# JTtNinjaCode/CPU-Ray-Tracing-Implementation

Hardware: AMD Instinct MI355X
Metric: Msamples/sec (pixels*spp) Cornell Box 800x800@1024spp; 1/2/4/8-GPU scaling (higher is better)
Workload: dtype fp64; 1 GPU; cornell_box 800x800 1024spp depth 50, light sampling on; key=cornell_box 800x800 1024spp depth 50 f64 pool=0 chunk=0 K=0 world=1, spp=1024, max_depth=50, tiles=16x16 round-robin over ranks, parallelism=tiles1, kernel_timing=on, rounds_per_frame=1, grid_lanes=458752

## Files before the change

### cpu-ray-tracing-implementation_amd/csrc/rt_device.h

```cpp
#pragma once

#include <hip/hip_runtime.h>
#include <stdint.h>

#include <type_traits>

#include "rt_room.h"
#include "rt_scene.h"
#include "rt_sin.h"
#include "rt_types.h"

namespace rtd {

#ifndef RT_BIG_SPHERE_R
#define RT_BIG_SPHERE_R 16
#endif
#define RT_EXT_FN __device__ __attribute__((noinline))

#ifndef RT_PRECISE_F32
__device__ __forceinline__ float fdiv(float a, float b) { return a * __builtin_amdgcn_rcpf(b); }
__device__ __forceinline__ float fsqrt(float x) { return __builtin_amdgcn_sqrtf(x); }
__device__ __forceinline__ float flog(float x) { return __builtin_amdgcn_logf(x) * 0.693147180559945309f; }
__device__ __forceinline__ float frsq(float x) { return __builtin_amdgcn_rsqf(x); }
__device__ __forceinline__ void sincos2pi(float u, float& s, float& c) {
// ... 7 lines not shown
__device__ __forceinline__ float frsq(float x) { return 1.0f / sqrtf(x); }
__device__ __forceinline__ void sincos2pi(float u, float& s, float& c) {
  float phi = 2 * 3.14159265358979f * u;
  s = sinf(phi);
  c = cosf(phi);
}
#endif
__device__ __forceinline__ double frcp(double b) {
  const double r0 = __builtin_amdgcn_rcp(b);
  double r = r0;
  double e = fma(-b, r, 1.0);
  r = fma(r, e, r);
  e = fma(-b, r, 1.0);
  r = fma(r, e, r);
  return __builtin_isfinite(r) ? r : r0;
}
__device__ __forceinline__ double fdiv(double a, double b) {
  const double r = frcp(b);
  const double q = a * r;
  const double res = fma(fma(-b, q, a), r, q);
  return __builtin_isfinite(res) ? res : q;
}
__device__ __forceinline__ double fdiv_fin(double a, double b) {
  const double r = frcp(b);
  const double q = a * r;
  return fma(fma(-b, q, a), r, q);
}
__device__ __forceinline__ double frsq(double x) {
  const double r0 = __builtin_amdgcn_rsq(x);
  const double h = 0.5 * x;
  double r = r0;
  r = r * fma(-h * r, r, 1.5);
  r = r * fma(-h * r, r, 1.5);
  return __builtin_isfinite(r) ? r : r0;
}
__device__ __forceinline__ double frsq_nz(double x) {
  const double r0 = __builtin_amdgcn_rsq(x);
  const double h = 0.5 * x;
  double r = r0;
  r = r * fma(-h * r, r, 1.5);
  r = r * fma(-h * r, r, 1.5);
  return r;
}
__device__ __forceinline__ double fsqrt01(double x) {
  const double r = __builtin_amdgcn_rsq(x);
  double g = x * r, h = 0.5 * r;
  const double e = fma(-g, h, 0.5);
  g = fma(g, e, g);
  h = fma(h, e, h);
  g = fma(fma(-g, g, x), h, g);
  return x > 0.0 ? g : 0.0;
}
__device__ __forceinline__ float fsqrt01(float x) { return fsqrt(x); }
__device__ __forceinline__ double fsqrt(double x) {
  const double r = __builtin_amdgcn_rsq(x);
  double g = x * r, h = 0.5 * r;
  const double e = fma(-g, h, 0.5);
  g = fma(g, e, g);
  h = fma(h, e, h);
  g = fma(fma(-g, g, x), h, g);
  return (x > 0.0 && x < __builtin_huge_val()) ? g : (x >= 0.0 ? x : __builtin_nan(""));
}
__device__ __forceinline__ float fdiv_inv(float a, float b, float inv_b) {
#ifndef RT_PRECISE_F32
  return a * inv_b;
#else
  return a / b;
#endif
}
__device__ __forceinline__ double fdiv_inv(double a, double b, double) { return fdiv(a, b); }
__device__ __forceinline__ double flog(double x) { return log(x); }
__device__ double2 g_sincos_tab[kSinCosTab];
__device__ __forceinline__ void sincos2pi(double u, double& s, double& c) {
  const double t = u * double(kSinCosTab);
  const double h = floor(t);
  const double2 sc = g_sincos_tab[(uint32_t)(int32_t)h & (kSinCosTab - 1)];
  const double d = (t - h) * (2.0 * 3.14159265358979323846 / kSinCosTab);
  const double d2 = d * d;
  const double sd = d * fma(d2, fma(d2, 1.0 / 120.0, -1.0 / 6.0), 1.0);
  const double cm1 = d2 * fma(d2, fma(d2, -1.0 / 720.0, 1.0 / 24.0), -0.5);
  s = fma(sc.y, sd, fma(sc.x, cm1, sc.x));
  c = fma(-sc.x, sd, fma(sc.y, cm1, sc.y));
}
__device__ __forceinline__ float div_pi(float x) { return fdiv(x, 3.14159265358979323846f); }
__device__ __forceinline__ double div_pi(double x) { return x * 0.318309886183790671537767526745; }
__device__ __forceinline__ float pow5(float x) { return (x * x) * (x * x) * x; }
__device__ __forceinline__ double pow5(double x) { return (x * x) * (x * x) * x; }

template <class R>
__device__ __forceinline__ V<R> mkv(R x, R y, R z) {
  return {x, y, z};
}
template <class R>
__device__ __forceinline__ V<R> ld3(const R* p) {
  return {p[0], p[1], p[2]};
}
template <class R>
__device__ __forceinline__ V<R> operator+(V<R> a, V<R> b) {
  return {a.x + b.x, a.y + b.y, a.z + b.z};
}
template <class R>
__device__ __forceinline__ V<R> operator-(V<R> a, V<R> b) {
  return {a.x - b.x, a.y - b.y, a.z - b.z};
}
template <class R>
__device__ __forceinline__ V<R> operator-(V<R> a) {
// ... 1215 lines not shown
  tmax = h ? th : tmax;
  best = h ? idx : best;
}
template <int A, class R>
__device__ __forceinline__ void flat_quads(const FlatQuadT<R>* q, uint32_t n, int32_t base, V<R> o, V<R> d,
                                           V<R> inv, R tmin, R& tmax, int32_t& best, uint64_t xkey) {
#pragma unroll 1
  for (uint32_t k = 0; k + 1 < n; k += 2) {
    const FlatQuad2<R> r = ld_scalar(reinterpret_cast<const FlatQuad2<R>*>(q + k));
    flat_quad_test<A>(r.a, base + (int32_t)k, o, d, inv, tmin, tmax, best, xkey);
    flat_quad_test<A>(r.b, base + (int32_t)k + 1, o, d, inv, tmin, tmax, best, xkey);
  }
  if (n & 1u) flat_quad_test<A>(ld_scalar(q + (n - 1)), base + (int32_t)(n - 1), o, d, inv, tmin, tmax, best, xkey);
}
template <class R>
struct Slab {
  R t0[3], t1[3], tn, tf, th;
};
template <class R>
__device__ __forceinline__ Slab<R> flat_slab(const FlatBoxT<R>& b, V<R> o, V<R> inv, R tmin, int32_t excl_i,
                                             uint32_t xf) {
  Slab<R> s;
  const bool left = sizeof(R) == 4 && excl_i == b.inst;
  const R ninf = -Num<R>::inf();
  auto dist = [&](R p, R oa, R ia) { return (p - oa) * ia; };
  s.t0[0] = (left & (xf == 0)) ? ninf : dist(b.lo[0], o.x, inv.x);
  s.t1[0] = (left & (xf == 1)) ? ninf : dist(b.hi[0], o.x, inv.x);
  s.t0[1] = (left & (xf == 2)) ? ninf : dist(b.lo[1], o.y, inv.y);
  s.t1[1] = (left & (xf == 3)) ? ninf : dist(b.hi[1], o.y, inv.y);
  s.t0[2] = (left & (xf == 4)) ? ninf : dist(b.lo[2], o.z, inv.z);
  s.t1[2] = (left & (xf == 5)) ? ninf : dist(b.hi[2], o.z, inv.z);
  s.tn = fmax(fmax(fmin(s.t0[0], s.t1[0]), fmin(s.t0[1], s.t1[1])), fmin(s.t0[2], s.t1[2]));
  s.tf = fmin(fmin(fmax(s.t0[0], s.t1[0]), fmax(s.t0[1], s.t1[1])), fmax(s.t0[2], s.t1[2]));
  s.th = s.tn >= tmin ? s.tn : s.tf;
  return s;
}
template <class R>
__device__ __forceinline__ RoomHit<R> flat_room_test(const FlatRoomHeadT<R>& b, V<R> o, V<R> inv, R tmin,
                                                     uint32_t excl_e, int32_t excl_i) {
  auto dist = [&](R p, R oa, R ia) { return (p - oa) * ia; };
  R t0[3] = {dist(b.lo[0], o.x, inv.x), dist(b.lo[1], o.y, inv.y), dist(b.lo[2], o.z, inv.z)};
  R t1[3] = {dist(b.hi[0], o.x, inv.x), dist(b.hi[1], o.y, inv.y), dist(b.hi[2], o.z, inv.z)};
  if constexpr (sizeof(R) == 4) {
    const bool left = excl_i == b.inst;
    const R ninf = -Num<R>::inf();
#pragma unroll
    for (int k = 0; k < 3; k++) {
      t0[k] = (left & (excl_e == b.e[2 * k]) & ((b.present >> (2 * k)) & 1u)) ? ninf : t0[k];
      t1[k] = (left & (excl_e == b.e[2 * k + 1]) & ((b.present >> (2 * k + 1)) & 1u)) ? ninf : t1[k];
    }
  }
  return room_rule<R>(t0, t1, b.present, tmin);
}
template <class R>
__device__ __forceinline__ void trace_flat(const DevScene<R>& sc, V<R> o, V<R> d, uint32_t excl_e, int32_t excl_i,
                                           R& t_best, uint32_t& e_best, int32_t& i_best, uint32_t& nm,
                                           const FlatQuadT<R>* fq, const FlatRoomT<R>* fr, const FlatBoxT<R>* fb) {
  const R tmin = R(0.001);
  R tmax = Num<R>::inf();
  const V<R> inv = flat_inv(d);
  const uint64_t xkey = ((uint64_t)(uint32_t)excl_i << 32) | excl_e;
  const uint32_t xf = excl_e & 7u;
  int32_t best = -1;
  const uint32_t n0 = sc.n_flatq[0], n1 = sc.n_flatq[1], n2 = sc.n_flatq[2], nq = n0 + n1 + n2;
  flat_quads<0>(sc.flatq, n0, 0, o, d, inv, tmin, tmax, best, xkey);
  flat_quads<1>(sc.flatq + n0, n1, (int32_t)n0, o, d, inv, tmin, tmax, best, xkey);
  flat_quads<2>(sc.flatq + n0 + n1, n2, (int32_t)(n0 + n1), o, d, inv, tmin, tmax, best, xkey);
  const uint32_t nr8 = (sizeof(R) == 8 || kFlatRoomsF32) ? 8u * sc.n_flatr : 0u;
  const FlatRoomT<R>* rooms = flat_rooms(sc);
#pragma unroll 1
  for (uint32_t k = 0; k < nr8; k += 8u) {
    const FlatRoomHeadT<R> b = ld_scalar(reinterpret_cast<const FlatRoomHeadT<R>*>(rooms + (k >> 3)));
    const RoomHit<R> r = flat_room_test(b, o, inv, tmin, excl_e, excl_i);
    const bool h = r.hit & (r.t <= tmax);
    tmax = h ? r.t : tmax;
    best = h ? (int32_t)(nq + k) + r.face : best;
  }
#pragma unroll 1
  for (uint32_t k = 0; k < sc.n_flatb; k++) {
    const FlatBoxT<R> b = ld_scalar(sc.flatb + k);
    const Slab<R> s = flat_slab(b, o, inv, tmin, excl_i, xf);
    const bool h = (s.tf >= fmax(s.tn, tmin)) & (s.th <= tmax);
    tmax = h ? s.th : tmax;
    best = h ? (int32_t)(nq + nr8 + k) : best;
  }
  t_best = tmax;
  e_best = kNoHit;
  i_best = -1;
  nm = 0;
  if (best < 0) return;
  if ((uint32_t)best < nq) {
    const FlatQuadT<R>& r = fq[best];
    e_best = r.e;
    i_best = r.inst;
    nm = r.nm;
    return;
  }
  if ((uint32_t)best < nq + nr8) {
    const uint32_t j = (uint32_t)best - nq;
    const FlatRoomT<R>& r = fr[j >> 3];
    e_best = r.e[j & 7u];
    i_best = r.inst;
    nm = r.nm[j & 7u];
    return;
  }
  const FlatBoxT<R>& b = fb[(uint32_t)best - nq - nr8];
  const Slab<R> s = flat_slab(b, o, inv, tmin, excl_i, xf);
  const bool enter = s.tn >= tmin;
  int k = 2;
  if (enter) {
    if (s.tn == fmin(s.t0[0], s.t1[0])) k = 0;
    else if (s.tn == fmin(s.t0[1], s.t1[1])) k = 1;
  } else {
    if (s.tf == fmax(s.t0[0], s.t1[0])) k = 0;
    else if (s.tf == fmax(s.t0[1], s.t1[1])) k = 1;
  }
  const R dk = k == 0 ? d.x : (k == 1 ? d.y : d.z);
  const int side = enter ? (dk < R(0) ? 1 : 0) : (dk < R(0) ? 0 : 1);
  e_best = b.face[2 * k + side];
  i_best = b.inst;
  nm = b.mat | (uint32_t)k << 28 | ((b.neg >> (2 * k + side)) & 1u) << 31;
}

__device__ __forceinline__ double perlin_noise(const double* tb, double px, double py, double pz) {
#pragma clang fp contract(off)
  int iu = (int)floor(px), iv = (int)floor(py), iw = (int)floor(pz);
  const double u = px - iu, v = py - iv, w = pz - iw;
  iu &= 255;
  iv &= 255;
  iw &= 255;
  const double* perm = tb + 3 * kPerlinPoints;
  const double uu = u * u * (3 - 2 * u), vv = v * v * (3 - 2 * v), ww = w * w * (3 - 2 * w);
  double accum = 0.0;
  for (int i = 0; i < 2; i++)
    for (int j = 0; j < 2; j++)
      for (int k = 0; k < 2; k++) {
        const int g = (int)perm[(iu + i) % 256] ^ (int)perm[(iv + j) % 256] ^ (int)perm[(iw + k) % 256];
        const double* r = tb + 3 * g;
        const double d = r[0] * (u - i) + r[1] * (v - j) + r[2] * (w - k);
        accum += (i * uu + (1 - i) * (1 - uu)) * (j * vv + (1 - j) * (1 - vv)) * (k * ww + (1 - k) * (1 - ww)) * d;
      }
  return accum;
}
RT_EXT_FN double perlin_texture(const double* tb, double scale, double px, double py, double pz) {
#pragma clang fp contract(off)
  double qx = px / scale, qy = py / scale, qz = pz / scale;
  double accum = 0, weight = 1.0;
  for (int i = 0; i < 7; i++) {
    accum += weight * perlin_noise(tb, qx, qy, qz);
    weight *= 0.5;
    qx *= 2.0;
    qy *= 2.0;
    qz *= 2.0;
  }
  return .5 * (1 + sin(px + 70 * fabs(accum)));
}
RT_EXT_FN double value_noise(const double* tb, uint32_t n, double px, double py, double pz) {
#pragma clang fp contract(off)
  const double fx = floor(px), fy = floor(py), fz = floor(pz);
  const double nn = (double)n, n3 = nn * nn * nn;
  auto at = [&](double ix, double iy, double iz) -> double {
    const double k = ix * nn * nn + iy * nn + iz;
    return (k >= 0 && k < n3) ? (double)(float)tb[(size_t)k] : 0.0;
  };
  const double x000 = at(fx, fy, fz), x100 = at(fx + 1, fy, fz), x010 = at(fx, fy + 1, fz),
               x110 = at(fx + 1, fy + 1, fz), x001 = at(fx, fy, fz + 1), x101 = at(fx + 1, fy, fz + 1),
               x011 = at(fx, fy + 1, fz + 1), x111 = at(fx + 1, fy + 1, fz + 1);
  const double x = px - fx, y = py - fy, z = pz - fz;
// ... 77 lines not shown
struct Onb {
  V<R> x, y, z;
};
template <class R>
__device__ __forceinline__ Onb<R> make_onb(V<R> n) {
  Onb<R> b;
  b.y = unit(n);
  if constexpr (sizeof(R) == 4) {
    const bool ez = fabsf(b.y.x) > 0.9f;
    const float c0 = ez ? b.y.y : 0.f, c1 = ez ? -b.y.x : b.y.z, c2 = ez ? 0.f : -b.y.y;
    const float r = frsq(ez ? c0 * c0 + c1 * c1 : c1 * c1 + c2 * c2);
    b.z = mkv(c0 * r, c1 * r, c2 * r);
  } else {
    V<R> a = (fabs(b.y.x) > R(0.9)) ? mkv(R(0), R(0), R(1)) : mkv(R(1), R(0), R(0));
    b.z = unit(cross(b.y, a));
  }
  b.x = cross(b.y, b.z);
  return b;
}
template <class R>
__device__ __forceinline__ Onb<R> make_onb_axis(V<R> n) {
  Onb<R> b;
  b.y = n;
  if constexpr (sizeof(R) == 4) {
    const bool ez = fabsf(b.y.x) > 0.9f;
    b.z = mkv(ez ? b.y.y : 0.f, ez ? -b.y.x : b.y.z, ez ? 0.f : -b.y.y);
  } else {
    const V<R> a = (fabs(b.y.x) > R(0.9)) ? mkv(R(0), R(0), R(1)) : mkv(R(1), R(0), R(0));
    b.z = cross(b.y, a);
  }
  b.x = cross(b.y, b.z);
  return b;
}
template <class R>
__device__ __forceinline__ V<R> onb_transform(const Onb<R>& b, V<R> v) {
  V<R> r = mkv(R(0), R(0), R(0));
  r = r + v.x * b.x;
  r = r + v.y * b.y;
  r = r + v.z * b.z;
  return r;
}
template <class R>
__device__ __forceinline__ V<R> on_sphere_sc(R u1, R sp, R cp) {
  R cos_theta = R(1) - R(2) * u1;
  R sin_theta = fsqrt01(R(1) - cos_theta * cos_theta);
  return mkv(sin_theta * cp, cos_theta, sin_theta * sp);
}
template <class R>
__device__ __forceinline__ V<R> on_sphere(R u1, R u2) {
  R sp, cp;
  sincos2pi(u2, sp, cp);
  return on_sphere_sc(u1, sp, cp);
}
template <class R>
__device__ __forceinline__ V<R> cosine_dir_sc(R r2, R sp, R cp) {
  R sr2 = fsqrt01(r2);
  return mkv(cp * sr2, fsqrt01(R(1) - r2), sp * sr2);
}
template <class R>
__device__ __forceinline__ V<R> cosine_dir(R r1, R r2) {
  R sp, cp;
  sincos2pi(r1, sp, cp);
  return cosine_dir_sc(r2, sp, cp);
}

template <class R>
struct R4s {
  R v[4];
};
template <class R>
struct LightUV {
  R u[3], pad1, v[3], pad2;
};
template <class R>
struct LightAF {
  R f[8];
};
template <int A, int U, int W>
__device__ __forceinline__ double light_pdf_aligned(const double* f, V<double> o, V<double> d) {
  const double rA = frcp(comp<A>(d));
  const double th = (f[0] - comp<A>(o)) * rA;
  if (!(0.001 <= th)) return 0.0;
  const double a = ((comp<U>(o) + th * comp<U>(d)) - f[1]) * f[3];
  const double b = ((comp<W>(o) + th * comp<W>(d)) - f[2]) * f[4];
  if (!(0.0 <= a && a <= 1.0 && 0.0 <= b && b <= 1.0)) return 0.0;
  const double dd = d.x * d.x + d.y * d.y + d.z * d.z;
  return ((th * th) * dd) * (dd * frsq_nz(dd)) * fabs(rA) * f[7];
}
template <class R, bool SEL = false>
__device__ __forceinline__ R light_pdf(const Light<R>* Lp, V<R> o, V<R> dir, bool sampled = false) {
  const int32_t kind = ld_here(&Lp->kind);
  if (kind == L_QUAD) {
    R t;
    bool hit;
    const int32_t aligned = ld_here(&Lp->aligned);
    if constexpr (sizeof(R) == 8) {
      if (aligned) {
        const LightAF<R> af = ld_here(reinterpret_cast<const LightAF<R>*>(Lp->af));
        switch (aligned) {
          case 1: return light_pdf_aligned<2, 0, 1>(af.f, o, dir);
          case 2: return light_pdf_aligned<1, 0, 2>(af.f, o, dir);
          case 3: return light_pdf_aligned<2, 1, 0>(af.f, o, dir);
          case 4: return light_pdf_aligned<0, 1, 2>(af.f, o, dir);
          case 5: return light_pdf_aligned<1, 2, 0>(af.f, o, dir);
          default: return light_pdf_aligned<0, 2, 1>(af.f, o, dir);
        }
      }
    }
    if (sizeof(R) == 4 && sampled && !(SEL && aligned)) {
      t = R(1);
      hit = true;
    } else if (aligned) {
      const LightAF<R> af = ld_here(reinterpret_cast<const LightAF<R>*>(Lp->af));
      const V<R> inv = rcp3(dir);
      switch (aligned) {
        case 1: hit = aquad_t<2, 0, 1>(af.f, o, dir, inv, R(0.001), Num<R>::inf(), t); break;
// ... 44 lines not shown
```

### cpu-ray-tracing-implementation_amd/csrc/rt_kernels.hip

```cpp
#include <hip/hip_runtime.h>

#include <algorithm>
#include <cmath>
#include <map>
#include <mutex>
#include <tuple>

#include "../../include/rt_hip.h"
#include "rt_device.h"
#include "rt_launch.h"

using namespace rtd;

namespace {

#ifndef RT_LINEAR_WAVES
#define RT_LINEAR_WAVES 6
#endif
#ifndef RT_STACK_WAVES
#define RT_STACK_WAVES 4
#endif
#ifndef RT_LINEAR_WAVES_F64
#define RT_LINEAR_WAVES_F64 3
#endif
#ifndef RT_STACK_WAVES_F64
#define RT_STACK_WAVES_F64 4
#endif
#ifndef RT_LINEAR_VOL_WAVES
#define RT_LINEAR_VOL_WAVES 6
#endif
#ifndef RT_LINEAR_VOL_WAVES_LLI
#define RT_LINEAR_VOL_WAVES_LLI 7
#endif
#ifndef RT_LINEAR_VOL_WAVES_F64
#define RT_LINEAR_VOL_WAVES_F64 4
#endif
constexpr uint32_t kQBatch = 64;
constexpr uint32_t kNoItem = 0xFFFFFFFFu;

constexpr uint32_t kDimDisk = 0x7FFF0000u, kDiskTries = 64;

template <class R>
struct Params : LaunchParams<R> {};

constexpr int kColdWords = 8, kColdDoubles = 3;
__device__ __forceinline__ uint32_t* cold_words() {
  __shared__ uint32_t w[kColdWords * kBlock];
  return w + threadIdx.x;
}
__device__ __forceinline__ double* cold_doubles() {
  __shared__ double w[kColdDoubles * kBlock];
  return w + threadIdx.x;
}
template <class R>
__device__ __forceinline__ R* cold_thr() {
  __shared__ R w[3 * kBlock];
  return w + threadIdx.x;
}
__device__ __forceinline__ __attribute__((unused)) double* cold_acc64() {
// ... 481 lines not shown
        has_add = true;
      }
      done = true;
    } else {
      V<R> att = LL ? col : tex_sample<R, CAMX>(sc, m.tx, pw, hu, hv);
      const uint32_t bounce = (uint32_t)s.bounce;
      uint32_t js = 0;
      auto U = [&]() { return to_unit<R>(draw_u32(s.ks, dim_scatter(bounce, js++))); };
      [[maybe_unused]] R nl_u1 = R(0), nl_u2 = R(0), nl_sp = R(0), nl_cp = R(0);
      constexpr bool kNlTrig = NL;
      if constexpr (kNlTrig) {
        nl_u1 = to_unit<R>(draw_u32(s.ks, dim_scatter(bounce, 0)));
        nl_u2 = to_unit<R>(draw_u32(s.ks, dim_scatter(bounce, 1)));
        sincos2pi(m.kind == M_METAL ? nl_u2 : nl_u1, nl_sp, nl_cp);
      }
      if (!LL && m.kind == M_METAL) {
        V<R> dir = unit(reflect(d, n));
        if constexpr (kNlTrig) {
          new_d = dir + m.fuzz * unit(on_sphere_sc(nl_u1, nl_sp, nl_cp));
        } else {
          R u1 = U();
          R u2 = U();
          new_d = dir + m.fuzz * unit(on_sphere(u1, u2));
        }
        s.set_thr(s.thr() * att);
      } else if (!LL && m.kind == M_DIELECTRIC) {
        R ri = front ? fdiv(R(1), m.refr) : m.refr;
        V<R> ud = unit(d);
        R cos_t = fmin(dot(-ud, n), R(1));
        R sin_t = fsqrt(R(1) - cos_t * cos_t);
        bool cant = ri * sin_t > R(1);
        R r0 = fdiv(R(1) - ri, R(1) + ri);
        r0 = r0 * r0;
        if (cant || (r0 + (R(1) - r0) * pow5(R(1) - cos_t)) > (kNlTrig ? nl_u1 : U()))
          new_d = reflect(ud, n);
        else
          new_d = refract(ud, n, ri);
        s.set_thr(s.thr() * att);
      } else if (!LL && !NL && m.kind == M_GLOSS && to_unit<R>(draw_u32(s.ks, dim_scatter(bounce, js))) <= m.spec) {
        js++;
        const Onb<R> b = FLAT ? make_onb_axis(n) : make_onb(n);
        const R r1 = U();
        const R r2 = U();
        const V<R> diffuse = onb_transform(b, cosine_dir(r1, r2));
        const R tt = m.smooth;
        new_d = unit((R(1) - tt) * diffuse + tt * reflect(d, n));
      } else {
        if (!LL && !NL && m.kind == M_GLOSS) js++;
        const bool iso = LL ? (LLI && ll_iso) : (!NL && m.kind == M_ISOTROPIC);
        const R iso_pdf = R(1) / (R(4) * Num<R>::pi());
        Onb<R> b;
        if (!FLAT && !iso) b = make_onb(n);
        auto cos_dir = [&](R u1, R u2) -> V<R> {
          const V<R> v = cosine_dir(u1, u2);
          if constexpr (FLAT) {
            const R sy = fs * v.y, sz = fs * v.z;
            return fA == 0 ? mkv(sy, -sz, -v.x) : (fA == 1 ? mkv(-v.x, sy, -sz) : mkv(-v.x, sz, sy));
          } else {
            return onb_transform(b, v);
          }
        };
        auto cos_n = [&](V<R> u) -> R {
          if constexpr (FLAT) return fs * (fA == 0 ? u.x : (fA == 1 ? u.y : u.z));
          return dot(u, b.y);
        };
        const Light<R>* Lt = sc.light;
        R pv = R(1);
        V<R> dir;
        bool own_pdf = false;
        if (NL || (!LL && ld_here(&Lt->kind) == L_NONE)) {
          if constexpr (kNlTrig) {
            dir = onb_transform(b, cosine_dir_sc(nl_u2, nl_sp, nl_cp));
          } else {
            R u1 = U();
            R u2 = U();
            dir = iso ? unit(on_sphere(u1, u2)) : cos_dir(u1, u2);
          }
          own_pdf = iso || unit_n;
          if (!own_pdf) pv = fmax(R(0), div_pi(cos_n(unit(dir))));
        } else {
          R c = U();
          R u1 = U();
          R u2 = U();
          const bool from_light = c < R(0.5);
          if constexpr (kMixSel) {
            const V<R> dl = light_random(Lt, pw, u1, u2);
            const V<R> dc = iso ? unit(on_sphere(u1, u2)) : cos_dir(u1, u2);
            dir = from_light ? dl : dc;
          } else if (from_light) {
            dir = light_random(Lt, pw, u1, u2);
          } else if constexpr (LLI) {
            R sp, cp;
            sincos2pi(iso ? u2 : u1, sp, cp);
            dir = iso ? unit(on_sphere_sc(u1, sp, cp)) : onb_transform(b, cosine_dir_sc(u2, sp, cp));
          } else {
            dir = iso ? unit(on_sphere(u1, u2)) : cos_dir(u1, u2);
          }
          R mp = iso ? iso_pdf : fmax(R(0), div_pi(cos_n(unit(dir))));
          pv = R(0.5) * light_pdf<R, kMixSel>(Lt, pw, dir, from_light) + R(0.5) * mp;
        }
        if (own_pdf) {
          s.set_thr(s.thr() * att);
        } else {
          R ps;
          if (iso) {
            ps = iso_pdf;
          } else {
            R c = FLAT ? cos_n(unit(dir)) : dot(n, unit(dir));
// ... 38 lines not shown
    s.xi = inst;
    return true;
  }
  RT_WIDE_STAT(8);
  V<R> acc = s.acc();
  if constexpr (!PS::kNoRad) acc = acc + s.rad;
  [[maybe_unused]] bool retire = false;
  const uint32_t sample = s.sample() + 1;
  s.set_sample(sample);
  if (sample < send_of(p, s)) {
    s.set_acc(acc);
  } else {
    const uint32_t item = s.item();
#ifdef RT_ITEM_CLOCKS
    if (g_item_clk) g_item_clk[item] = (uint32_t)(wall_clock64() - s.t0_);
#endif
    R* dst = p.partial + 3ull * item;
    dst[0] = acc.x;
    dst[1] = acc.y;
    dst[2] = acc.z;
    s.set_acc(mkv(R(0), R(0), R(0)));
    const uint32_t nx = p.persist == kPersist ? next_item_dyn(p) : (item + p.P < p.n_items ? item + p.P : kNoItem);
    if (nx == kNoItem) {
      if constexpr (kInPlace) {
        retire = true;
      } else {
        s.bounce = -1;
        return false;
      }
    } else {
      begin_item(p, s, nx);
    }
  }
  begin_sample<R, CAMX>(p, s);
  if constexpr (kInPlace) {
    if (retire) {
      s.bounce = -1;
      return false;
    }
  }
  return true;
}

struct TravDefaults {
  static constexpr bool kFlat = false;
  static constexpr bool kWide = false;
  static constexpr bool kTablesLds = false;
  struct Tables {};
  static constexpr int kStack = 0;
  static constexpr int kLdsNodes = 0;
  static constexpr uint32_t kLdsMats = 16;
  [[maybe_unused]] static constexpr bool kLL = false, kNL = false, kLLI = false, kMoving = true;
  [[maybe_unused]] static constexpr bool kLean = false, kNoRad = false, kColdLds = false, kThrLds = false;
};
template <class R, bool SPH, bool TRI, bool VOL, bool LLI = false>
struct LinearTrav : TravDefaults {
  static constexpr bool kLL = LLI, kLLI = LLI;
  static constexpr int kWaves = sizeof(R) != 4 ? (VOL ? RT_LINEAR_VOL_WAVES_F64 : RT_LINEAR_WAVES_F64)
                                 : (!SPH && !TRI && !VOL) ? RT_LINEAR_WAVES
                                 : (!SPH && !TRI && VOL)  ? (LLI ? RT_LINEAR_VOL_WAVES_LLI : RT_LINEAR_VOL_WAVES)
                                                          : 1;
  static constexpr bool kNoRad = VOL;
  static constexpr bool kColdLds = VOL;
  static constexpr bool kThrLds = VOL && LLI && sizeof(R) == 4;
  template <class PS>
  __device__ __forceinline__ static void run(const DevScene<R>& sc, const Node<R>*, const PS& s, Keys k,
                                             uint32_t*, R& t, uint32_t& e, int32_t& i, uint32_t&) {
    trace_linear<R, SPH, TRI, VOL>(sc, s.o, s.d, s.tm, s.xe, s.xi, k, (uint32_t)s.bounce, t, e, i);
  }
};
#ifndef RT_FLAT_WAVES
#define RT_FLAT_WAVES 8
#endif
#ifndef RT_FLAT_WAVES_F64
#define RT_FLAT_WAVES_F64 5
#endif
#ifndef RT_FLAT_WAVES_F64_LL
#define RT_FLAT_WAVES_F64_LL 7
#endif
template <class R, bool TLDS = false, bool LL = false>
struct FlatTrav : TravDefaults {
  static constexpr bool kFlat = true;
  static constexpr bool kTablesLds = TLDS;
  static constexpr bool kLL = LL;
  static constexpr int kWaves = sizeof(R) == 4 ? RT_FLAT_WAVES : (LL ? RT_FLAT_WAVES_F64_LL : RT_FLAT_WAVES_F64);
  static constexpr bool kNoRad = true;
  static constexpr bool kColdLds = sizeof(R) == 8;
  template <class PS>
  __device__ __forceinline__ static void run(const DevScene<R>& sc, const Node<R>*, const PS& s, Keys, uint32_t*,
                                             R& t, uint32_t& e, int32_t& i, uint32_t& nm) {
    trace_flat<R>(sc, s.o, s.d, s.xe, s.xi, t, e, i, nm, sc.flatq, flat_rooms(sc), sc.flatb);
  }
  static constexpr uint32_t kLdsQuads = LL ? 14 : 64, kLdsBoxes = LL ? 8 : 16, kLdsMats = LL ? 16 : 32;
  static constexpr uint32_t kLdsRooms = LL ? 1 : 2;
  struct Tables {
    FlatQuadT<R> q[kLdsQuads];
    FlatRoomT<R> r[kLdsRooms];
    FlatBoxT<R> b[kLdsBoxes];
    Material<R> m[LL ? 1 : kLdsMats];
    R4<R> lm[LL ? kLdsMats : 1];
  };
  __host__ __device__ __forceinline__ static bool tables_fit(const DevScene<R>& sc) {
    return sc.n_flatq[0] + sc.n_flatq[1] + sc.n_flatq[2] <= kLdsQuads && sc.n_flatb <= kLdsBoxes &&
           sc.n_flatr <= kLdsRooms && sc.n_mats <= kLdsMats;
  }
  __device__ __forceinline__ static void fill(const DevScene<R>& sc, Tables& tb) {
    const uint32_t nq = sc.n_flatq[0] + sc.n_flatq[1] + sc.n_flatq[2];
    for (uint32_t j = threadIdx.x; j < nq; j += kBlock) tb.q[j] = sc.flatq[j];
    if constexpr (sizeof(R) == 8 || kFlatRoomsF32)
      for (uint32_t j = threadIdx.x; j < sc.n_flatr; j += kBlock) tb.r[j] = flat_rooms(sc)[j];
    for (uint32_t j = threadIdx.x; j < sc.n_flatb; j += kBlock) tb.b[j] = sc.flatb[j];
    for (uint32_t j = threadIdx.x; j < sc.n_mats; j += kBlock) {
      if constexpr (LL) {
        const Material<R>& m = sc.mats[j];
        tb.lm[j] = R4<R>{m.tx.c0[0], m.tx.c0[1], m.tx.c0[2], m.kind == M_DIFFUSE_LIGHT ? R(1) : R(0)};
      } else {
        tb.m[j] = sc.mats[j];
      }
    }
  }
  template <class PS>
  __device__ __forceinline__ static void run_lds(const DevScene<R>& sc, const Tables& tb, const PS& s, R& t,
                                                 uint32_t& e, int32_t& i, uint32_t& nm) {
    trace_flat<R>(sc, s.o, s.d, s.xe, s.xi, t, e, i, nm, tb.q, tb.r, tb.b);
  }
};
constexpr uint32_t kLdsNodeMax = 256;
template <class R, int STACK, bool LDSN = false>
struct StackTrav : TravDefaults {
  static constexpr int kStack = STACK;
  static constexpr int kLdsNodes = LDSN ? (int)kLdsNodeMax : 0;
  static constexpr int kWaves = sizeof(R) == 4 ? RT_STACK_WAVES : (LDSN ? 1 : RT_STACK_WAVES_F64);
  template <class PS>
  __device__ __forceinline__ static void run(const DevScene<R>& sc, const Node<R>* nodes, const PS& s, Keys k,
                                             uint32_t* stk, R& t, uint32_t& e, int32_t& i, uint32_t&) {
    trace<R, STACK, kBlock>(sc, LDSN ? nodes : sc.nodes, s.o, s.d, s.tm, s.xe, s.xi, k, (uint32_t)s.bounce, s.xy(),
                            stk, t, e, i);
  }
};

#ifndef RT_WIDE_WAVES
#define RT_WIDE_WAVES 7
#endif
#ifndef RT_SHADE_BATCH
#define RT_SHADE_BATCH 48
#endif
#ifndef RT_SHADE_BATCH_GLOBAL
#define RT_SHADE_BATCH_GLOBAL 48
#endif
#ifndef RT_WIDE_WAVES_F64
#define RT_WIDE_WAVES_F64 4
#endif
#ifndef RT_WIDE_WAVES_GLOBAL_F64
#define RT_WIDE_WAVES_GLOBAL_F64 4
#endif
#ifndef RT_WIDE_WAVES_GLOBAL_F64_LL
#define RT_WIDE_WAVES_GLOBAL_F64_LL 5
#endif
#ifndef RT_WIDE_WAVES_F64_NL
#define RT_WIDE_WAVES_F64_NL 5
#endif
template <class R, bool SPH, bool TRI, bool QUAD, bool MOV, bool LDSN, bool LL = false, bool NL = false>
struct WideTrav : TravDefaults {
  static constexpr bool kWide = true;
  static constexpr bool kLL = LL, kNL = NL, kMoving = MOV;
  static constexpr int kWaves = sizeof(R) == 4 ? (LDSN ? RT_WIDE_WAVES : RT_WIDE_WAVES_GLOBAL)
                                               : (LDSN ? (NL ? RT_WIDE_WAVES_F64_NL : RT_WIDE_WAVES_F64)
                                                       : (LL ? RT_WIDE_WAVES_GLOBAL_F64_LL : RT_WIDE_WAVES_GLOBAL_F64));
  static constexpr bool kThrLds = sizeof(R) == 8 && !LDSN && LL;
  static constexpr bool kLean = true;
  static constexpr bool kNoRad = true;
  using StackT = WStackT<LDSN>;
  using WW = typename WWord<R>::T;
  __host__ __device__ static uint32_t stack_offset(uint32_t n_wnodes, uint32_t n_words) {
    return LDSN ? n_wnodes * kWNodeLdsStride + n_words * (uint32_t)sizeof(WW) : 0u;
  }
  static constexpr bool kTop = !LDSN && sizeof(R) == 4;
// ... 98 lines not shown
  R4<R> Dv{};
  if (active) {
    slot = p.queue ? p.queue[i] : i;
    Dv = p.D[slot];
    active = Dv.w >= R(0);
  }
  if (active) {
    Path<R> s;
    load_path(p, slot, Dv, s);
#ifdef RT_SECTION_CLOCKS
    uint64_t c_trace = 0, c_shade = 0, c_store = 0;
#endif
#pragma unroll 1
    for (int k = 0; k < p.K; k++) {
      R t;
      uint32_t e, nm = 0;
      int32_t inst;
      RT_LANE_TIMED(c_trace, Trav::run(p.sc, lds_nodes, s, Keys{s.ks}, stk.v + threadIdx.x, t, e, inst, nm));
      segs++;
      if (!RT_LANE_TIMED(c_shade, shade<R, CAMX, ShadeGeneral<Trav::kFlat>>(p, s, t, e, inst, nm))) break;
    }
    RT_LANE_TIMED(c_store, store_path(p, slot, s));
#ifdef RT_SECTION_CLOCKS
    atomicAdd(&g_section_clocks[0], (unsigned long long)c_trace);
    atomicAdd(&g_section_clocks[1], (unsigned long long)c_shade);
    atomicAdd(&g_section_clocks[2], (unsigned long long)c_store);
    atomicAdd(&g_section_clocks[3], 1ull);
#endif
  }
  for (int off = 32; off > 0; off >>= 1) segs += __shfl_xor(segs, off);
  if ((threadIdx.x & 63) == 0) wave_cnt[threadIdx.x >> 6] = segs;
  __syncthreads();
  if (threadIdx.x == 0) {
    uint32_t c = wave_cnt[0] + wave_cnt[1] + wave_cnt[2] + wave_cnt[3];
    if (c) atomicAdd(&p.seg_shards[blockIdx.x % kSegShards], (unsigned long long)c);
  }
}

template <class R>
__device__ __forceinline__ const Params<R>& reload_params() {
  using KP = const __attribute__((address_space(4))) Params<R>*;
  KP kp = (KP)__builtin_amdgcn_kernarg_segment_ptr();
  asm volatile("" : "+s"(kp));
  return *(const Params<R>*)kp;
}
template <class R>
__device__ __forceinline__ bool seg_cap_hit(const Params<R>& q, uint64_t segs) {
  if (segs > q.seg_cap) {
    atomicOr(q.fault, 1u);
    return true;
  }
  return false;
}
template <class R, class Trav, bool CAMX>
__device__ __forceinline__ void persist_body(const Params<R>& p) {
  __shared__ Lds<Trav::kStack * kBlock> stk;
  __shared__ uint32_t wave_cnt[kBlock / 64];
  __shared__ Node<R> lds_nodes[Trav::kLdsNodes > 0 ? Trav::kLdsNodes : 1];
  if constexpr (Trav::kLdsNodes > 0) {
    for (uint32_t j = threadIdx.x; j < p.sc.n_nodes; j += kBlock) lds_nodes[j] = p.sc.nodes[j];
    __syncthreads();
  }
  uint32_t* stk_lane = stk.v + threadIdx.x;
  const Node<R>* trav_nodes = lds_nodes;
  [[maybe_unused]] void* wstk = nullptr;
#ifdef RT_SECTION_CLOCKS
  if (threadIdx.x < 10) wide_stats_lds()[threadIdx.x] = 0;
  __syncthreads();
#endif
  if constexpr (Trav::kWide) {
    extern __shared__ uint4 dyn_lds[];
    wstk = Trav::fill(p.sc, dyn_lds) + threadIdx.x;
    trav_nodes = (const Node<R>*)dyn_lds;
  }
  const Material<R>* mats = nullptr;
  const R4<R>* lm = nullptr;
  [[maybe_unused]] const typename Trav::Tables* flat_tb = nullptr;
  if constexpr (Trav::kTablesLds) {
    __shared__ typename Trav::Tables tb;
    Trav::fill(p.sc, tb);
    __syncthreads();
    flat_tb = &tb;
    mats = tb.m;
    lm = tb.lm;
  }
  if constexpr (Trav::kLL && !Trav::kTablesLds) {
    __shared__ R4<R> wlm_tab[Trav::kLdsMats];
    for (uint32_t j = threadIdx.x; j < p.sc.n_mats; j += kBlock) {
      const Material<R>& m = p.sc.mats[j];
      wlm_tab[j] = R4<R>{m.tx.c0[0], m.tx.c0[1], m.tx.c0[2],
                         m.kind == M_DIFFUSE_LIGHT ? R(1) : (m.kind == M_ISOTROPIC ? R(2) : R(0))};
    }
    __syncthreads();
    lm = wlm_tab;
  }
  uint32_t item0 = blockIdx.x * kBlock + threadIdx.x;
  if (p.persist == kPersist) {
    if ((threadIdx.x & 63) == 0) {
      __hip_atomic_store(wave_queue(), 0u, __ATOMIC_RELAXED, __HIP_MEMORY_SCOPE_WAVEFRONT);
      __hip_atomic_store(wave_queue() + 1, 0u, __ATOMIC_RELAXED, __HIP_MEMORY_SCOPE_WAVEFRONT);
    }
    item0 = next_item_dyn(p);
  }
  uint64_t segs = 0;
  if (item0 < p.n_items) {
    Path<R, Trav::kColdLds, Trav::kLean, Trav::kNoRad, Trav::kThrLds> s;
    s.set_acc(mkv(R(0), R(0), R(0)));
    begin_item(p, s, item0);
    begin_sample<R, CAMX>(p, s);
    if constexpr (Trav::kWide) {
      using StackT = typename Trav::StackT;
      const uint32_t root = Trav::root(p.sc);
      WideRayT<R> ry{root, 0, Num<R>::inf(), kNoHit, 1u};
#pragma unroll 1
      for (;;) {
        const Params<R>& q = reload_params<R>();
        if (!RT_WAVE_TIMED(6, Trav::steps(q.sc, trav_nodes, s, (StackT*)wstk, ry))) continue;
        if (seg_cap_hit(q, ++segs)) break;
        const R t = ry.tmax;
        const uint32_t e = ry.e;
        ry = WideRayT<R>{root, 0, Num<R>::inf(), kNoHit, 1u};
        RT_WIDE_STAT(4);
        if (!RT_WAVE_TIMED(7, shade<R, CAMX, ShadeOf<Trav>>(q, s, t, e, -1, 0, mats, lm))) break;
      }
    } else {
#pragma unroll 1
      for (;;) {
        const Params<R>& q = reload_params<R>();
        R t;
        uint32_t e, nm = 0;
        int32_t inst;
        RT_WIDE_STAT(0);
        if constexpr (Trav::kTablesLds)
          RT_WAVE_TIMED(6, Trav::run_lds(q.sc, *flat_tb, s, t, e, inst, nm));
        else
          RT_WAVE_TIMED(6, Trav::run(q.sc, trav_nodes, s, Keys{s.ks}, stk_lane, t, e, inst, nm));
        if (seg_cap_hit(q, ++segs)) break;
        if (!RT_WAVE_TIMED(7, shade<R, CAMX, ShadeOf<Trav>>(q, s, t, e, inst, nm, mats, lm))) break;
      }
    }
  }
  uint32_t sg = (uint32_t)segs;
  for (int off = 32; off > 0; off >>= 1) sg += __shfl_xor(sg, off);
  if ((threadIdx.x & 63) == 0) wave_cnt[threadIdx.x >> 6] = sg;
  __syncthreads();
  if (threadIdx.x == 0) {
    uint64_t c = (uint64_t)wave_cnt[0] + wave_cnt[1] + wave_cnt[2] + wave_cnt[3];
    if (c) atomicAdd(&p.seg_shards[blockIdx.x % kSegShards], (unsigned long long)c);
  }
#ifdef RT_SECTION_CLOCKS
  if (threadIdx.x < 10) atomicAdd(&g_wide_stats[threadIdx.x], wide_stats_lds()[threadIdx.x]);
#endif
}
template <class R, class Trav, bool CAMX>
__global__ __launch_bounds__(kBlock) void k_persist(Params<R> p) {
  persist_body<R, Trav, CAMX>(p);
}
#ifndef RT_CAMX_WAVES
#define RT_CAMX_WAVES 4
#endif
#ifndef RT_CAMX_WAVES_F64
#define RT_CAMX_WAVES_F64 2
#endif
#define RT_CAMX_W(R) (sizeof(R) == 8 ? RT_CAMX_WAVES_F64 : RT_CAMX_WAVES)
template <class R, class Trav, bool CAMX>
__global__ __launch_bounds__(kBlock) __attribute__((amdgpu_waves_per_eu(CAMX ? RT_CAMX_W(R) : Trav::kWaves))) void k_persist_occ(
    Params<R> p) {
  persist_body<R, Trav, CAMX>(p);
}

template <class R, class Trav, bool CAMX>
__global__ __launch_bounds__(kBlock) void k_step(Params<R> p) {
  step_body<R, Trav, CAMX>(p);
}
template <class R, class Trav, bool CAMX>
__global__ __launch_bounds__(kBlock) __attribute__((amdgpu_waves_per_eu(CAMX ? RT_CAMX_W(R) : Trav::kWaves))) void k_step_occ(Params<R> p) {
  step_body<R, Trav, CAMX>(p);
}

template <class R>
struct KTrace : TraceParams<R> {};

template <class R>
struct QueryRay {
  V<R> o, d;
  R tm;
  int32_t bounce;
  uint32_t ks;
  uint32_t xe;
  int32_t xi;
  __device__ __forceinline__ uint32_t xy() const { return 0u; }
// ... 410 lines not shown
    s2 = s2 / inv;
  }
  out[3ull * px] = s0;
  out[3ull * px + 1] = s1;
  out[3ull * px + 2] = s2;
}

template <class R>
__global__ void k_zero(R* out, uint64_t n) {
  uint64_t i = blockIdx.x * (uint64_t)kBlock + threadIdx.x;
  if (i < n) out[i] = R(0);
}

__global__ __launch_bounds__(kBlock) void k_pixmap(const uint4* tl, uint32_t ntiles, uint32_t npix, uint32_t* pixmap) {
  const uint32_t i = blockIdx.x * kBlock + threadIdx.x;
  if (i >= npix) return;
  uint32_t lo = 0, hi = ntiles - 1;
  while (lo < hi) {
    const uint32_t mid = (lo + hi + 1) >> 1;
    if (tl[mid].w <= i) lo = mid;
    else hi = mid - 1;
  }
  const uint4 t = tl[lo];
  const uint32_t k = i - t.w, y = k / t.z, x = k - y * t.z;
  pixmap[i] = (t.x + x) | (t.y + y) << 16;
}


std::mutex g_occ_mu;
std::map<std::tuple<const void*, int, size_t>, uint32_t> g_occ;

uint32_t resident_blocks(const void* kern, int dev, size_t lds) {
  std::lock_guard<std::mutex> lk(g_occ_mu);
  auto it = g_occ.find({kern, dev, lds});
  if (it != g_occ.end()) return it->second;
  int n = 0, b = 0;
  uint32_t r = 0;
  if (hipDeviceGetAttribute(&n, hipDeviceAttributeMultiprocessorCount, dev) == hipSuccess &&
      hipOccupancyMaxActiveBlocksPerMultiprocessor(&b, kern, kBlock, lds) == hipSuccess && b > 0 && n > 0)
    r = (uint32_t)(b * n);
  g_occ[{kern, dev, lds}] = r;
  return r;
}

thread_local uint64_t t_grid_lanes = 0;

template <class KernelT, class R>
void launch_one(KernelT kern, Params<R> p, uint32_t grid, hipStream_t st, size_t lds = 0) {
  if (p.persist) {
    int dev = 0;
    const uint32_t res = hipGetDevice(&dev) == hipSuccess ? resident_blocks((const void*)kern, dev, lds) : 0;
    if (res > 0) grid = std::min<uint32_t>(grid, res);
    p.P = grid * kBlock;
    p.seg_cap = (uint64_t)p.n_items * p.chunk * (uint64_t)p.max_depth + 1;
    t_grid_lanes = (uint64_t)grid * kBlock;
  }
  hipLaunchKernelGGL(kern, dim3(grid), dim3(kBlock), lds, st, p);
}

static_assert(((size_t)RT_WIDE_LDS_STACK * kBlock * 4u + (size_t)RT_WIDE_TOP_N * kWTopStride + 1024u) *
                      RT_WIDE_WAVES_GLOBAL <= (160u << 10),
              "RT_WIDE_LDS_STACK / RT_WIDE_TOP_N do not fit RT_WIDE_WAVES_GLOBAL blocks per CU");
static_assert(((size_t)RT_WIDE_LDS_STACK_F64 * kBlock * 4u + (size_t)RT_WIDE_TOP_N_F64 * sizeof(WNodeH) +
               3u * kBlock * sizeof(double) + 1024u) *
                      RT_WIDE_WAVES_GLOBAL_F64_LL <= (160u << 10),
              "RT_WIDE_LDS_STACK_F64 / RT_WIDE_TOP_N_F64 do not fit RT_WIDE_WAVES_GLOBAL_F64_LL blocks per CU");
static_assert(RT_WIDE_TOP_N <= kWideTopMax && RT_WIDE_TOP_N_F64 <= kWideTopMax,
              "the scene compiler orders at most kWideTopMax top nodes first");
template <class R>
inline size_t wide_lds_bytes(const DevScene<R>& sc, bool ldsn) {
  const size_t stack = ldsn ? (size_t)sc.wide_stack * kBlock * 2u
                            : (size_t)std::min<uint32_t>(sc.wide_stack, wide_lds_stack<R>()) * kBlock * 4u;
  const size_t top = (!ldsn && sizeof(R) == 4)
                         ? (size_t)std::min<uint32_t>(sc.wide_top, RT_WIDE_TOP_N) * kWTopStride
                     : (!ldsn && sizeof(R) == 8)
                         ? (size_t)std::min<uint32_t>(sc.wide_top, RT_WIDE_TOP_N_F64) * sizeof(WNodeH) : 0u;
  if (ldsn) return wide_lds_tree_bytes(sc.n_wnodes, sc.n_wprim_words, sc.wide_stack, sizeof(typename WWord<R>::T));
  return stack + top;
}
template <class R, bool SPH, bool TRI, bool QUAD, bool MOV, bool LL = false, bool NL = false>
void launch_wide_k(const Params<R>& p, uint32_t grid, hipStream_t st) {
  const size_t full = wide_lds_bytes(p.sc, true);
  const uint32_t spill_grid = p.sc.wide_spill ? std::min<uint32_t>(grid, p.sc.spill_lanes / kBlock) : grid;
  if (wide_tree_in_lds(p.sc.n_wnodes, p.sc.n_wprim_words, p.sc.wide_stack, sizeof(typename WWord<R>::T))) {
    launch_one(k_persist_occ<R, WideTrav<R, SPH, TRI, QUAD, MOV, true, LL, NL>, false>, p, grid, st, full);
    return;
  }
  launch_one(k_persist_occ<R, WideTrav<R, SPH, TRI, QUAD, MOV, false, LL, NL>, false>, p, spill_grid, st,
             wide_lds_bytes(p.sc, false));
}
template <class R>
inline void launch_wide(const Params<R>& p, bool ll, bool nl, uint32_t grid, hipStream_t st) {
  const uint32_t k = p.sc.wide_kinds;
  if (k == WK_SPHERE && nl)
    launch_wide_k<R, true, false, false, false, false, true>(p, grid, st);
  else if (k == WK_SPHERE)
    launch_wide_k<R, true, false, false, false>(p, grid, st);
  else if (k == WK_TRI)
    launch_wide_k<R, false, true, false, false>(p, grid, st);
  else if (k == (WK_TRI | WK_QUAD) && ll && p.sc.n_mats <= 16)
    launch_wide_k<R, false, true, true, false, true>(p, grid, st);
  else if (k == (WK_TRI | WK_QUAD))
    launch_wide_k<R, false, true, true, false>(p, grid, st);
  else
    launch_wide_k<R, true, true, true, true>(p, grid, st);
}
template <class R, class Trav>
// ... 248 lines not shown
```

### cpu-ray-tracing-implementation_amd/csrc/rt_room.h

```cpp
#pragma once

#include <math.h>
#include <stdint.h>

#if !defined(__HIP__) && !defined(__host__)
#define __host__
#define __device__
#endif

namespace rtd {

constexpr uint32_t kRoomAllFaces = 63u;

__host__ __device__ inline uint32_t room_absent(uint32_t present) {
  uint32_t f = 0;
  while (f < 6u && ((present >> f) & 1u)) f++;
  return f;
}
__host__ __device__ inline bool room_mask_ok(uint32_t present) {
  const uint32_t miss = ~present & kRoomAllFaces;
  return (present & ~kRoomAllFaces) == 0 && (miss & (miss - 1u)) == 0;
}

template <class R>
struct RoomHit {
  bool hit;
  R t;
  int face;
};

template <class R>
__host__ __device__ inline RoomHit<R> room_rule(const R t0[3], const R t1[3], uint32_t present, R tmin) {
  const R n0 = fmin(t0[0], t1[0]), n1 = fmin(t0[1], t1[1]), n2 = fmin(t0[2], t1[2]);
  const R f0 = fmax(t0[0], t1[0]), f1 = fmax(t0[1], t1[1]), f2 = fmax(t0[2], t1[2]);
  const R tn = fmax(fmax(n0, n1), n2);
  const R tf = fmin(fmin(f0, f1), f2);
  bool in_absent = false, out_absent = false;
  switch (room_absent(present)) {
    case 0: in_absent = tn == t0[0], out_absent = tf == t0[0]; break;
    case 1: in_absent = tn == t1[0], out_absent = tf == t1[0]; break;
    case 2: in_absent = tn == t0[1], out_absent = tf == t0[1]; break;
    case 3: in_absent = tn == t1[1], out_absent = tf == t1[1]; break;
    case 4: in_absent = tn == t0[2], out_absent = tf == t0[2]; break;
    case 5: in_absent = tn == t1[2], out_absent = tf == t1[2]; break;
    default: break;
  }
  const bool enter = (tn >= tmin) & !in_absent;
  RoomHit<R> r;
  r.hit = (tf >= fmax(tn, tmin)) & (enter | !out_absent);
  r.t = enter ? tn : tf;
  const bool l0 = t0[0] == r.t, h0 = t1[0] == r.t, l1 = t0[1] == r.t, h1 = t1[1] == r.t, h2 = t1[2] == r.t;
  const bool a0 = l0 | h0, a1 = l1 | h1;
  const bool hi = (a0 & h0) | (!a0 & a1 & h1) | (!a0 & !a1 & h2);
  r.face = (a0 ? 0 : (a1 ? 2 : 4)) + (hi ? 1 : 0);
  return r;
}

}
```

Baseline: 27540 Msamples/s.

## Encode box hit axis during traversal, trim fp64 sqrt and sign ops, narrow segment counter

For fp64 flat-scene traversal, the box loop now records the entering axis in the best index, so the closing box slab recomputation is skipped for entering hits. The fp64 cosine-direction sampling uses a square root without the zero-clamp select and flips signs with an XOR instead of a multiply. The segment counter becomes 32-bit when possible (the cap is clamped to UINT32_MAX), and the cap check moves after shading for most traversals. Together these cut ALU work per bounce, in exchange for extra face-rule work inside the box loop and a slight change in when the cap aborts.

```diff
diff --git a/cpu-ray-tracing-implementation_amd/csrc/rt_device.h b/cpu-ray-tracing-implementation_amd/csrc/rt_device.h
--- a/cpu-ray-tracing-implementation_amd/csrc/rt_device.h
+++ b/cpu-ray-tracing-implementation_amd/csrc/rt_device.h
@@ -83,6 +83,18 @@
   return x > 0.0 ? g : 0.0;
 }
 __device__ __forceinline__ float fsqrt01(float x) { return fsqrt(x); }
+__device__ __forceinline__ double fsqrt01_nz(double x) {
+  const double r = __builtin_amdgcn_rsq(x);
+  double g = x * r, h = 0.5 * r;
+  const double e = fma(-g, h, 0.5);
+  g = fma(g, e, g);
+  h = fma(h, e, h);
+  return fma(fma(-g, g, x), h, g);
+}
+__device__ __forceinline__ float fsqrt01_nz(float x) { return fsqrt(x); }
+__device__ __forceinline__ double flip_sign(double x, bool neg) {
+  return __longlong_as_double(__double_as_longlong(x) ^ (neg ? (long long)0x8000000000000000ull : 0ll));
+}
 __device__ __forceinline__ double fsqrt(double x) {
   const double r = __builtin_amdgcn_rsq(x);
   double g = x * r, h = 0.5 * r;
@@ -1404,7 +1416,7 @@
   }
   return room_rule<R>(t0, t1, b.present, tmin);
 }
-template <class R>
+template <class R, bool FACE = false>
 __device__ __forceinline__ void trace_flat(const DevScene<R>& sc, V<R> o, V<R> d, uint32_t excl_e, int32_t excl_i,
                                            R& t_best, uint32_t& e_best, int32_t& i_best, uint32_t& nm,
                                            const FlatQuadT<R>* fq, const FlatRoomT<R>* fr, const FlatBoxT<R>* fb) {
@@ -1434,7 +1446,12 @@
     const Slab<R> s = flat_slab(b, o, inv, tmin, excl_i, xf);
     const bool h = (s.tf >= fmax(s.tn, tmin)) & (s.th <= tmax);
     tmax = h ? s.th : tmax;
-    best = h ? (int32_t)(nq + nr8 + k) : best;
+    if constexpr (FACE) {
+      const BoxFaceHit<R> f = box_face_rule<R>(s.t0, s.t1, tmin);
+      best = h ? (int32_t)(nq + nr8 + 4u * k) + (f.enter ? f.axis : 3) : best;
+    } else {
+      best = h ? (int32_t)(nq + nr8 + k) : best;
+    }
   }
   t_best = tmax;
   e_best = kNoHit;
@@ -1456,16 +1473,27 @@
     nm = r.nm[j & 7u];
     return;
   }
-  const FlatBoxT<R>& b = fb[(uint32_t)best - nq - nr8];
-  const Slab<R> s = flat_slab(b, o, inv, tmin, excl_i, xf);
-  const bool enter = s.tn >= tmin;
+  const uint32_t bj = (uint32_t)best - nq - nr8;
+  const FlatBoxT<R>& b = fb[FACE ? bj >> 2 : bj];
+  bool enter;
   int k = 2;
-  if (enter) {
-    if (s.tn == fmin(s.t0[0], s.t1[0])) k = 0;
-    else if (s.tn == fmin(s.t0[1], s.t1[1])) k = 1;
+  if constexpr (FACE) {
+    enter = (bj & 3u) != 3u;
+    k = (int)(bj & 3u);
+    if (!enter) {
+      const Slab<R> s = flat_slab(b, o, inv, tmin, excl_i, xf);
+      k = box_face_rule<R>(s.t0, s.t1, tmin).axis;
+    }
   } else {
-    if (s.tf == fmax(s.t0[0], s.t1[0])) k = 0;
-    else if (s.tf == fmax(s.t0[1], s.t1[1])) k = 1;
+    const Slab<R> s = flat_slab(b, o, inv, tmin, excl_i, xf);
+    enter = s.tn >= tmin;
+    if (enter) {
+      if (s.tn == fmin(s.t0[0], s.t1[0])) k = 0;
+      else if (s.tn == fmin(s.t0[1], s.t1[1])) k = 1;
+    } else {
+      if (s.tf == fmax(s.t0[0], s.t1[0])) k = 0;
+      else if (s.tf == fmax(s.t0[1], s.t1[1])) k = 1;
+    }
   }
   const R dk = k == 0 ? d.x : (k == 1 ? d.y : d.z);
   const int side = enter ? (dk < R(0) ? 1 : 0) : (dk < R(0) ? 0 : 1);
@@ -1649,16 +1677,16 @@
   sincos2pi(u2, sp, cp);
   return on_sphere_sc(u1, sp, cp);
 }
-template <class R>
+template <class R, bool DRAW = false>
 __device__ __forceinline__ V<R> cosine_dir_sc(R r2, R sp, R cp) {
   R sr2 = fsqrt01(r2);
-  return mkv(cp * sr2, fsqrt01(R(1) - r2), sp * sr2);
-}
-template <class R>
+  return mkv(cp * sr2, DRAW ? fsqrt01_nz(R(1) - r2) : fsqrt01(R(1) - r2), sp * sr2);
+}
+template <class R, bool DRAW = false>
 __device__ __forceinline__ V<R> cosine_dir(R r1, R r2) {
   R sp, cp;
   sincos2pi(r1, sp, cp);
-  return cosine_dir_sc(r2, sp, cp);
+  return cosine_dir_sc<R, DRAW>(r2, sp, cp);
 }
 
 template <class R>
diff --git a/cpu-ray-tracing-implementation_amd/csrc/rt_kernels.hip b/cpu-ray-tracing-implementation_amd/csrc/rt_kernels.hip
--- a/cpu-ray-tracing-implementation_amd/csrc/rt_kernels.hip
+++ b/cpu-ray-tracing-implementation_amd/csrc/rt_kernels.hip
@@ -5,6 +5,7 @@
 #include <map>
 #include <mutex>
 #include <tuple>
+#include <type_traits>
 
 #include "../../include/rt_hip.h"
 #include "rt_device.h"
@@ -592,8 +593,11 @@
         Onb<R> b;
         if (!FLAT && !iso) b = make_onb(n);
         auto cos_dir = [&](R u1, R u2) -> V<R> {
-          const V<R> v = cosine_dir(u1, u2);
-          if constexpr (FLAT) {
+          const V<R> v = cosine_dir<R, FLAT && LL>(u1, u2);
+          if constexpr (FLAT && LL && sizeof(R) == 8) {
+            const R sy = flip_sign(v.y, fs < R(0)), sz = flip_sign(v.z, fs < R(0));
+            return fA == 0 ? mkv(sy, -sz, -v.x) : (fA == 1 ? mkv(-v.x, sy, -sz) : mkv(-v.x, sz, sy));
+          } else if constexpr (FLAT) {
             const R sy = fs * v.y, sz = fs * v.z;
             return fA == 0 ? mkv(sy, -sz, -v.x) : (fA == 1 ? mkv(-v.x, sy, -sz) : mkv(-v.x, sz, sy));
           } else {
@@ -738,6 +742,7 @@
   static constexpr uint32_t kLdsMats = 16;
   [[maybe_unused]] static constexpr bool kLL = false, kNL = false, kLLI = false, kMoving = true;
   [[maybe_unused]] static constexpr bool kLean = false, kNoRad = false, kColdLds = false, kThrLds = false;
+  static constexpr bool kCapBeforeShade = false;
 };
 template <class R, bool SPH, bool TRI, bool VOL, bool LLI = false>
 struct LinearTrav : TravDefaults {
@@ -749,6 +754,7 @@
   static constexpr bool kNoRad = VOL;
   static constexpr bool kColdLds = VOL;
   static constexpr bool kThrLds = VOL && LLI && sizeof(R) == 4;
+  static constexpr bool kCapBeforeShade = VOL && LLI && sizeof(R) == 4;
   template <class PS>
   __device__ __forceinline__ static void run(const DevScene<R>& sc, const Node<R>*, const PS& s, Keys k,
                                              uint32_t*, R& t, uint32_t& e, int32_t& i, uint32_t&) {
@@ -808,7 +814,7 @@
   template <class PS>
   __device__ __forceinline__ static void run_lds(const DevScene<R>& sc, const Tables& tb, const PS& s, R& t,
                                                  uint32_t& e, int32_t& i, uint32_t& nm) {
-    trace_flat<R>(sc, s.o, s.d, s.xe, s.xi, t, e, i, nm, tb.q, tb.r, tb.b);
+    trace_flat<R, sizeof(R) == 8>(sc, s.o, s.d, s.xe, s.xi, t, e, i, nm, tb.q, tb.r, tb.b);
   }
 };
 constexpr uint32_t kLdsNodeMax = 256;
@@ -1013,6 +1019,14 @@
   }
   return false;
 }
+template <class R>
+__device__ __forceinline__ bool seg_cap_hit(const Params<R>& p, const Params<R>& q, uint32_t segs) {
+  if (segs > (uint32_t)q.seg_cap) {
+    atomicOr(p.fault, 1u);
+    return true;
+  }
+  return false;
+}
 template <class R, class Trav, bool CAMX>
 __device__ __forceinline__ void persist_body(const Params<R>& p) {
   __shared__ Lds<Trav::kStack * kBlock> stk;
@@ -1063,7 +1077,7 @@
     }
     item0 = next_item_dyn(p);
   }
-  uint64_t segs = 0;
+  std::conditional_t<Trav::kWide || Trav::kCapBeforeShade, uint64_t, uint32_t> segs = 0;
   if (item0 < p.n_items) {
     Path<R, Trav::kColdLds, Trav::kLean, Trav::kNoRad, Trav::kThrLds> s;
     s.set_acc(mkv(R(0), R(0), R(0)));
@@ -1096,8 +1110,12 @@
           RT_WAVE_TIMED(6, Trav::run_lds(q.sc, *flat_tb, s, t, e, inst, nm));
         else
           RT_WAVE_TIMED(6, Trav::run(q.sc, trav_nodes, s, Keys{s.ks}, stk_lane, t, e, inst, nm));
-        if (seg_cap_hit(q, ++segs)) break;
+        ++segs;
+        if constexpr (Trav::kCapBeforeShade)
+          if (seg_cap_hit(q, segs)) break;
         if (!RT_WAVE_TIMED(7, shade<R, CAMX, ShadeOf<Trav>>(q, s, t, e, inst, nm, mats, lm))) break;
+        if constexpr (!Trav::kCapBeforeShade)
+          if (seg_cap_hit(p, q, segs)) break;
       }
     }
   }
@@ -1614,7 +1632,7 @@
     const uint32_t res = hipGetDevice(&dev) == hipSuccess ? resident_blocks((const void*)kern, dev, lds) : 0;
     if (res > 0) grid = std::min<uint32_t>(grid, res);
     p.P = grid * kBlock;
-    p.seg_cap = (uint64_t)p.n_items * p.chunk * (uint64_t)p.max_depth + 1;
+    p.seg_cap = std::min<uint64_t>((uint64_t)p.n_items * p.chunk * (uint64_t)p.max_depth + 1, UINT32_MAX);
     t_grid_lanes = (uint64_t)grid * kBlock;
   }
   hipLaunchKernelGGL(kern, dim3(grid), dim3(kBlock), lds, st, p);
diff --git a/cpu-ray-tracing-implementation_amd/csrc/rt_room.h b/cpu-ray-tracing-implementation_amd/csrc/rt_room.h
--- a/cpu-ray-tracing-implementation_amd/csrc/rt_room.h
+++ b/cpu-ray-tracing-implementation_amd/csrc/rt_room.h
@@ -56,4 +56,24 @@
   return r;
 }
 
+template <class R>
+struct BoxFaceHit {
+  R t;
+  int axis;
+  bool enter;
+};
+template <class R>
+__host__ __device__ inline BoxFaceHit<R> box_face_rule(const R t0[3], const R t1[3], R tmin) {
+  const R n0 = fmin(t0[0], t1[0]), n1 = fmin(t0[1], t1[1]), n2 = fmin(t0[2], t1[2]);
+  const R f0 = fmax(t0[0], t1[0]), f1 = fmax(t0[1], t1[1]), f2 = fmax(t0[2], t1[2]);
+  const R tn = fmax(fmax(n0, n1), n2);
+  const R tf = fmin(fmin(f0, f1), f2);
+  BoxFaceHit<R> r;
+  r.enter = tn >= tmin;
+  r.t = r.enter ? tn : tf;
+  const int an = tn == n0 ? 0 : (tn == n1 ? 1 : 2), af = tf == f0 ? 0 : (tf == f1 ? 1 : 2);
+  r.axis = r.enter ? an : af;
+  return r;
 }
+
+}
```

Result: faster. 28160 Msamples/s (median of 6 runs) (+2.2%).
